# urw7rs/diffusion-models-made-easy

Hardware: AMD Instinct MI355X
Metric: denoising steps/sec + training images/sec, DDPM UNet CIFAR10 32×32 @1/2/4/8 GPU (higher is better)
Workload: dtype bf16; 1 GPU; DDPM T=1000 sampling, CIFAR10 32x32, default UNet (32,416,643 params, random init), batch 128 per GPU, t.shape=(1,); global_batch=128, parallelism=dp1 (independent chains per GPU, no data-path collective)

## Files before the change

diffusion-models-made-easy_amd/_lib.py:

```python

from __future__ import annotations

import ctypes as C
import os
import subprocess
import threading

_HERE = os.path.dirname(os.path.abspath(__file__))
LIB_PATH = os.environ.get("DMME_LIB_PATH") or os.path.join(_HERE, "libdmme_hip.so")
CSRC = os.path.join(_HERE, "csrc")

F16R32 = 4
F32, BF16, BF16X3, F16 = 0, 1, 2, 3
CHAIN_DDPM, CHAIN_DDIM, CHAIN_IDDPM, CHAIN_DDPM_GUIDED, CHAIN_DDIM_GUIDED, CHAIN_GDDIM = 0, 1, 2, 3, 4, 5
CHAIN_DDPM_CFG, CHAIN_GDDIM_CFG = 6, 7
CHAIN_DPMPP, CHAIN_DPMPP_CFG = 8, 9
CHAIN_REPAINT = 10
CHAIN_ILVR = 11
PRED_EPS, PRED_X0, PRED_V = 0, 1, 2
PREDICTIONS = {"eps": PRED_EPS, "x0": PRED_X0, "v": PRED_V}
THRESHOLD_NONE, THRESHOLD_STATIC, THRESHOLD_DYNAMIC = 0, 1, 2
THRESHOLDS = {"none": THRESHOLD_NONE, "static": THRESHOLD_STATIC, "dynamic": THRESHOLD_DYNAMIC}
ARCH_DDPM, ARCH_IDDPM, ARCH_CLASSIFIER, ARCH_DDPM_COND = 0, 1, 2, 3
DTYPES = {"fp32": F32, "float32": F32, "32": F32, "bf16": BF16, "bfloat16": BF16, "16": BF16, "bf16-mixed": BF16, "16-mixed": BF16,
# ... 93 lines not shown
    "dmme_unet_plan_check": (_i, [_vp]),
    "dmme_debug_level_stamps": (_i, [_vp, _i, _i]),
    "dmme_unet_plan_op_info": (_i, [_vp, _i, C.c_char_p, _i, C.POINTER(C.c_double), C.POINTER(C.c_double)]),
    "dmme_unet_forward_profiled": (_i, [_vp, _vp, _vp, _vp, _i, _vp, _vp, _vp, _vp, _vp]),
    "dmme_unet_plan_packed_bwd_bytes": (_i64, [_vp]),
    "dmme_unet_plan_bwd_workspace_bytes": (_i64, [_vp]),
    "dmme_unet_pack_params_bwd": (_i, [_vp, _vp, _vp, _vp]),
    "dmme_unet_backward": (_i, [_vp, _vp, _vp, _vp, _vp, _i, _vp, _vp, _vp, _vp, _vp, _vp, _vp]),
    "dmme_unet_backward_buckets": (_i, [_vp, _vp, _vp, _vp, _vp, _i, _vp, _vp, _vp, _vp, _vp, _vp, _vp, BUCKET_FN, _vp]),
    "dmme_unet_backward_input": (_i, [_vp, _vp, _vp, _vp, _vp, _i, _vp, _vp, _vp, _vp, _vp, _vp]),
    "dmme_unet_plan_grad_buckets": (_i, [_vp, C.POINTER(_i64), C.POINTER(_i64), C.POINTER(_i), _i]),
    "dmme_unet_plan_bwd_summary": (_i, [_vp, C.c_char_p, _i]),
    "dmme_grad_norm": (_i, [_vp, _i64, _vp, _vp, _vp]),
    "dmme_adam_step": (_i, [_vp, _vp, _vp, _vp, _vp, _i64, _f, _f, _f, _f, _i, _vp, _f, _f, _f, _vp]),
    "dmme_amp_init": (_i, [_vp, _f, _vp]),
    "dmme_amp_scale": (_i, [_vp, _i64, _vp, _vp]),
    "dmme_adam_step_amp": (_i, [_vp, _vp, _vp, _vp, _vp, _i64, _f, _f, _f, _f, _vp, _f, _f, _f, _vp, _f, _f, _i, _vp]),
    "dmme_grad_pack_bf16": (_i, [_vp, _i64, _vp, _i64, _vp]),
    "dmme_shard_reduce_bf16": (_i, [_vp, _i, _i64, _f, _vp, _vp]),
    "dmme_grad_unpack_bf16": (_i, [_vp, _i64, _vp, _vp]),
    "dmme_unet_debug_read": (_i, [_vp, _vp, C.c_char_p, _vp, _i64, C.POINTER(_i64), _vp]),
    "dmme_unet_debug_read_grad": (_i, [_vp, _vp, C.c_char_p, _vp, _i64, C.POINTER(_i64), _vp]),
    "dmme_unet_debug_read_norm_stats": (_i, [_vp, _vp, C.c_char_p, _vp, _i64, C.POINTER(_i64), _vp]),
    "dmme_dropout_masks": (_i, [_vp, _u64, _u64, _vp, _vp]),
    "dmme_randn": (_i, [_vp, _i64, _u64, _u64, _vp]),
    "dmme_q_sample": (_i, [_vp, _vp, _vp, _vp, _vp, _i, _i64, _vp, _vp, _vp]),
    "dmme_ddpm_step": (_i, [_vp, _vp, _vp, _f, _f, _f, _i, _i64, _vp]),
    "dmme_ddim_step": (_i, [_vp, _vp, _f, _f, _i64, _vp]),
    "dmme_gddim_step": (_i, [_vp, _vp, _vp, _f, _f, _f, _i64, _vp]),
    "dmme_slerp": (_i, [_vp, _vp, _vp, _i, _i, _i64, _vp, _vp]),
    "dmme_chain_set": (_i, [_vp, _i64, _vp, _u64, _u64, _vp]),
    "dmme_chain_update": (_i, [_i, _vp, _vp, _vp, _vp, _vp, _i, _i64, _vp]),
    "dmme_chain_step": (_i, [_vp, _vp, _vp, _vp, _vp, _i, _vp, _vp, _vp, _vp]),
    "dmme_chain_update_gddim": (_i, [_vp, _vp, _vp, _vp, _vp, _vp, _i, _i64, _vp]),
    "dmme_log_softmax_grad": (_i, [_vp, _vp, _i, _i, _i, _f, _vp, _vp, _vp, _vp]),
    "dmme_chain_update_guided": (_i, [_i, _vp, _vp, _vp, _vp, _vp, _vp, _vp, _i, _i64, _vp]),
    "dmme_guided_chain_step": (_i, [_vp, _vp, _vp, _vp, _vp, _vp, _vp, _vp, _vp, _vp, _vp, _vp, _vp, _vp, _vp, _i, _vp, _vp, _vp, _vp]),
    "dmme_mse_loss": (_i, [_vp, _vp, _i64, _vp, _vp, _f, _vp, _vp]),
    "dmme_pred_to_eps": (_i, [_i, _vp, _vp, _vp, _i, _vp, _i, _i, _i64, _vp]),
    "dmme_unet_plan_set_prediction": (_i, [_vp, _i, _vp, _i]),
    "dmme_x0_threshold": (_i, [_i, _vp, _vp, _vp, _i, _vp, _i, _i, _i64, _i, _i, _f, _i, _f, _vp, _vp]),
    "dmme_x0_threshold_scratch_bytes": (_i64, [_i, _i64]),
    "dmme_x0_threshold_lds_capacity": (_i, []),
    "dmme_unet_plan_set_threshold": (_i, [_vp, _i, _vp, _i, _i, _f, _vp]),
    "dmme_q_sample_pred": (_i, [_i, _vp, _vp, _vp, _vp, _vp, _i, _i64, _vp, _vp, _vp]),
    "dmme_mse_loss_rows": (_i, [_vp, _vp, _vp, _vp, _i, _i64, _vp, _vp, _f, _vp, _vp]),
# ... 96 lines not shown
```

diffusion-models-made-easy_amd/csrc/common.h:

```cpp
#pragma once

#include <hip/hip_runtime.h>
#include <stdint.h>

#include "dmme_hip.h"

namespace dmme {

void set_error(const char* fmt, ...) __attribute__((format(printf, 1, 2)));

int debug_route(const char* key, int dflt = 0);

#define DMME_CHECK_HIP(expr)                                                                          \
    do {                                                                                              \
        hipError_t e_ = (expr);                                                                       \
        if (e_ != hipSuccess) {                                                                       \
            ::dmme::set_error("%s failed: %s (%s:%d)", #expr, hipGetErrorString(e_), __FILE__, __LINE__); \
            return DMME_ERR_HIP;                                                                      \
        }                                                                                             \
    } while (0)

#define DMME_REQUIRE(cond, code, ...)        \
    do {                                     \
        if (!(cond)) {                       \
// ... 148 lines not shown
    const void* res1;
    const void* res2;
    void* dst;
    int N, Hin, Win, C1, C2;
    int up, stride, taps;
    int Hout, Wout, Cout;
    int pro_silu, out_silu;
    int nt, tproj_ld, R1;
    int in_nchw, out_nchw;
    float* gn_part;
    int gn_cg, gn_tiles;
    int gn_raw_moments;
    long long* stamps;
    float* splitk;
    int64_t splitk_cap;
    int x3;
    int mix;
    int mix2;
    int f16;
    int dma_b;
    GnOut gno[2];
    int n_gno;
    float gn_eps;
    void* act;
    int act_k, act_silu;
    const float* act_dmask;
    GnIn gni;
    int has_gni;
    const void* r_src1;
    const void* r_src2;
    const void* r_w;
    const float* r_bias;
    int r_C1, r_C2;
};

int launch_mfma_valu(int mode, int iters, int blocks, float* sink, hipStream_t s);
int launch_issue_probe(int kind, int n_inner, int iters, int flags, int blocks, long long* sink, const void* src, hipStream_t s);
int launch_l2_stream(const void* buf, int64_t bytes, int iters, int mode, int depth, int blocks, unsigned* sink, hipStream_t s);

struct ConvTile {
    int TW, TH, TN;
    int HH, HWd;
    int tiles_x, tiles_y;
    int tiles_m, tiles_n;
    int a_rows;
    unsigned magic_px, magic_w;
};
enum ConvFamily {
    CONV_GENERIC = 0,
// ... 325 lines not shown
```

diffusion-models-made-easy_amd/csrc/conv_common.h:

```cpp
#pragma once
#include <stdlib.h>

#include "common.h"

namespace dmme {

typedef float f32x16 __attribute__((ext_vector_type(16)));
typedef float f32x4 __attribute__((ext_vector_type(4)));
typedef __bf16 bf16x8 __attribute__((ext_vector_type(8)));
typedef f16 f16x8 __attribute__((ext_vector_type(8)));
template <typename T>
struct Vec8 {
    typedef T type __attribute__((ext_vector_type(8)));
};
template <typename T>
__device__ __forceinline__ void unpack8(const uint4& raw, float (&v)[8]) {
    const typename Vec8<T>::type x = __builtin_bit_cast(typename Vec8<T>::type, raw);
#pragma unroll
    for (int e = 0; e < 8; ++e) v[e] = (float)x[e];
}
template <typename T>
__device__ __forceinline__ uint4 pack8(const float (&v)[8]) {
    typename Vec8<T>::type x;
#pragma unroll
// ... 779 lines not shown
            float na = 0.f, mean = 0.f, m2 = 0.f;
            for (int j = 0; j < f; ++j) {
                const float* q = img + (tn * VPR + gi * f + j) * 2;
                const float delta = q[0] - mean, tot = na + cv;
                const float rt = __builtin_amdgcn_rcpf(tot);
                mean += delta * (cv * rt);
                m2 += q[1] + delta * delta * (na * cv * rt);
                na = tot;
            }
            const float rstd = 1.0f / sqrtf(m2 / na + a.gn_eps);
            for (int j = 0; j < f; ++j) {
                float* o = mr + (k * 256 + tn * VPR + gi * f + j) * 2;
                o[0] = mean;
                o[1] = rstd;
            }
            if (n0 + tn < a.N && G.mean_rstd) {
                float* o = G.mean_rstd + ((int64_t)(n0 + tn) * (G.C / G.cg) + (G.c_off + co0) / G.cg + gi) * 2;
                o[0] = mean;
                o[1] = rstd;
            }
        }
    }
    __syncthreads();
    for (int idx = tid; idx < TN * BN; idx += NT) {
        const int tn = idx / BN, c = idx % BN;
#pragma unroll
        for (int k = 0; k < 2; ++k) {
            if (k >= a.n_gno) break;
            const GnOut& G = a.gno[k];
            const float* q = mr + (k * 256 + tn * VPR + c / VEC) * 2;
            const int cc = G.c_off + co0 + c;
            const float gm = idx == tid ? gm0[k] : G.gamma[cc], bt = idx == tid ? bt0[k] : G.beta[cc];
            const float sc = q[1] * gm, sh = bt - q[0] * sc;
            if (n0 + tn < a.N) {
                G.scale[(int64_t)(n0 + tn) * G.C + cc] = sc;
                G.shift[(int64_t)(n0 + tn) * G.C + cc] = sh;
            }
            if (a.act && k == a.act_k) {
                ssc[idx] = sc;
                ssh[idx] = sh;
            }
        }
    }
    if (!a.act) return;
    __syncthreads();
    const GnOut& GA = a.gno[a.act_k];
    T* __restrict__ act = (T*)a.act;
#pragma unroll
    for (int q = 0; q < ITEMS; ++q) {
        const int it = tid + q * NT, m = it / VPR;
        const int opix = pix_of(m);
        if (opix < 0) continue;
        const int tn = m >> sh_hw;
        const float* dm = a.act_dmask ? a.act_dmask + (int64_t)(n0 + tn) * GA.C + GA.c_off + co0 + vec * VEC : nullptr;
        const uint4 o = prologue_vec<T>(kept[q], ssc + tn * BN + vec * VEC, ssh + tn * BN + vec * VEC, dm, a.act_silu);
        *reinterpret_cast<uint4*>(act + (int64_t)opix * GA.C + GA.c_off + co0 + vec * VEC) = o;
    }
}

template <typename T, int BM, int BN, int MI, int NI, int NT = 256, typename PixFn>
__device__ __forceinline__ void conv_epilogue(const ConvArgs& a, f32x16 (&acc)[MI][NI], int co0, int wn0, int r, int h,
                                              int wm0, int n0, int TN, PixFn pix_of, float* stage, int tile_s) {
    if (conv_epilogue_is_staged<T>(a, TN)) {
        conv_epilogue_stage<T, BN, MI, NI>(a, acc, co0, wn0, r, h, wm0, n0, stage);
        __syncthreads();
        conv_epilogue_store<T, BM, BN, NT>(a, co0, n0, pix_of, stage, tile_s);
        return;
    }
#pragma unroll
    for (int ni = 0; ni < NI; ++ni) {
        const int co = co0 + wn0 + ni * 32 + r;
        if (co >= a.Cout) continue;
        const float bias = a.bias ? a.bias[co] : 0.f;
#pragma unroll
        for (int mi = 0; mi < MI; ++mi) {
#pragma unroll
            for (int j = 0; j < 16; ++j) {
                const int m = wm0 + mi * 32 + (j & 3) + 8 * (j >> 2) + 4 * h;
                const int opix = pix_of(m);
// ... 62 lines not shown
```

diffusion-models-made-easy_amd/csrc/plan.h:

```cpp
#pragma once
#include <stdarg.h>
#include <stdlib.h>
#include <stdio.h>
#include <string.h>

#include <algorithm>
#include <memory>
#include <string>
#include <unordered_map>
#include <vector>

#include "common.h"
#include "lvl.h"

namespace dmme {

static inline int64_t align_up(int64_t v, int64_t a) { return (v + a - 1) / a * a; }

template <typename T>
class DevTable {
    T* p_ = nullptr;

public:
    DevTable() = default;
// ... 65 lines not shown
    int64_t lin_pre = -1;
    int gn_src1 = -1, gn_src2 = -1, gn_gamma = -1, gn_beta = -1;
    int64_t b_rowsum = 0, b_ab = 0;
    int64_t b_gnrows = -1;
    int gn_rows_deferred = 0;
    int64_t gn_scale = 0, gn_shift = 0, gn_mr = 0;
    int gn_mod_col = -1, gn_mod_C = 0;
    int64_t gn_act = -1;
    int gn_force_small = 0;
    int gn_consumer = -1;
    int gn_direct = 0;
    int gn_in_consumer = 0;
    int src1 = -1, src2 = -1;
    int w = -1, b = -1;
    int gn = -1;
    int pro_silu = 0, out_silu = 0;
    int64_t dmask_off = -1;
    int tproj_col = -1;
    int res1 = -1, res2 = -1;
    int dst = -1;
    int up = 0, stride = 1, taps = 9;
    int use_act = 0;
    int gd_n = 0, gd_gn[2] = {-1, -1}, gd_coff[2] = {0, 0};
    int gd_act = -1;
    int res_alias = 0;
    int rseg = -1, fused_away = 0;
    int wg_layer = -1;
    int64_t wg_act = -1;
    int bias_deferred = 0;
    int at_qkv = -1, at_out = -1, at_heads = 1;
    int64_t at_lse = 0;
    int at_proj = -1;
    int at_fold_qkv = -1;
    int folded_into = -1;
    int64_t fold_M = -1, fold_c = -1, fold_wpv = -1, fold_b2 = -1;
    int mix = 0, route_f32 = 0;
    int mix2 = 0;
    int cast_src = -1, cast_dst = -1;
    int lvl = -1, lvl_first = 0;
};

struct LvlRun {
    int op_first = 0, op_last = 0;
    int sh = 0, NG = 0, NGS = 0, GB = 1, NJ = 1;
    std::vector<LvlOp> ops;
    std::vector<std::pair<int, int>> made;
    DevTable<LvlOp> ops_dev;
// ... 108 lines not shown
```

diffusion-models-made-easy_amd/csrc/plan.hip:

```cpp
#include "plan.h"

#include <functional>
#include <map>
#include <mutex>

namespace dmme {

static thread_local char g_err[512] = "";
void set_error(const char* fmt, ...) {
    va_list ap;
    va_start(ap, fmt);
    vsnprintf(g_err, sizeof(g_err), fmt, ap);
    va_end(ap);
}

int debug_route(const char* key, int dflt) {
    const char* e = getenv("DMME_DEBUG_ROUTE");
    if (!e || !*e) return dflt;
    const size_t kl = strlen(key);
    for (const char* p = e; *p;) {
        const char* end = strchr(p, ',');
        const size_t len = end ? (size_t)(end - p) : strlen(p);
        if (len >= kl && !strncmp(p, key, kl) && (len == kl || p[kl] == '=')) return len == kl ? 1 : atoi(p + kl + 1);
        if (!end) break;
// ... 645 lines not shown
        a.res1 = ws + P->tensors[o.res1].off;
        a.R1 = P->tensors[o.res1].C;
        if (o.res2 >= 0) a.res2 = ws + P->tensors[o.res2].off;
    }
    if (P->splitk_floats > 0 && ws) {
        a.splitk = (float*)(ws + P->ws_splitk);
        a.splitk_cap = P->splitk_floats;
    }
    if (fwd && o.gd_n > 0) {
        a.n_gno = o.gd_n;
        a.gn_eps = 1e-5f;
        a.gn_cg = P->tensors[o.dst].C / P->cfg.num_groups;
        for (int k = 0; k < o.gd_n; ++k) {
            const Op& g = P->ops[o.gd_gn[k]];
            GnOut& G = a.gno[k];
            G.gamma = (const float*)(packed + P->params[g.gn_gamma].packed_off);
            G.beta = (const float*)(packed + P->params[g.gn_beta].packed_off);
            G.scale = (float*)(ws + g.gn_scale);
            G.shift = (float*)(ws + g.gn_shift);
            G.mean_rstd = (float*)(ws + g.gn_mr);
            G.C = P->tensors[g.gn_src1].C + (g.gn_src2 >= 0 ? P->tensors[g.gn_src2].C : 0);
            G.cg = G.C / P->cfg.num_groups;
            G.c_off = o.gd_coff[k];
            if (k == o.gd_act) {
                const Op& cv = P->ops[g.gn_consumer];
                a.act = ws + g.gn_act;
                a.act_k = k;
                a.act_silu = cv.pro_silu;
                a.act_dmask = (cv.dmask_off >= 0 && drop_masks) ? drop_masks + cv.dmask_off : nullptr;
            }
        }
    }
    a.gn_raw_moments = P->mix ? 1 : 0;
    if (o.dst == -2) {
        a.dst = y;
        a.out_nchw = 1;
    } else {
        const Tensor& td = P->tensors[o.dst];
        a.dst = ws + td.off;
        if (td.stats_off >= 0) {
            a.gn_part = (float*)(ws + td.stats_off);
            a.gn_cg = td.C / P->cfg.num_groups;
            a.gn_tiles = td.stats_tiles;
        }
    }
}

bool gn_from_parts(const dmme_plan* P, const Op& o) {
    if (o.gn_force_small) return false;
    const Tensor& t1 = P->tensors[o.gn_src1];
    if (t1.stats_off < 0) return false;
    const int G = P->cfg.num_groups;
// ... 83 lines not shown
            }
        }
    }
    int64_t ws = P->ws_bytes;
    const int64_t es = (int64_t)dtype_size(P->dtype);
    for (int t = 0; t < nT; ++t) {
        if (!elig[t]) continue;
        Op& o = P->ops[producer[t]];
        P->tensors[t].stats_off = -1;
        o.gd_n = (int)uses[t].size();
        for (int k = 0; k < o.gd_n; ++k) {
            o.gd_gn[k] = uses[t][k].gn;
            o.gd_coff[k] = uses[t][k].coff;
            P->ops[uses[t][k].gn].gn_direct = 1;
        }
    }
    if (getenv("DMME_NO_PREACT")) return;
    for (int ci = 0; ci < nO; ++ci) {
        Op& cv = P->ops[ci];
        if (cv.kind != OP_CONV || cv.gn < 0 || cv.src1 < 0 || cv.up || cv.stride != 1 || cv.lvl >= 0) continue;
        Op& g = P->ops[cv.gn];
        if (!g.gn_direct || g.gn_src2 >= 0 || g.gn_act >= 0 || g.gn_src1 != cv.src1 || cv.src2 >= 0) continue;
        Op& pr = P->ops[producer[g.gn_src1]];
        if (pr.gd_act >= 0 || elig[g.gn_src1] != 1) continue;
        for (int k = 0; k < pr.gd_n; ++k)
            if (pr.gd_gn[k] == cv.gn) pr.gd_act = k;
        if (pr.gd_act < 0) continue;
        const Tensor& t1 = P->tensors[g.gn_src1];
        g.gn_act = ws;
        g.gn_consumer = ci;
        cv.use_act = 1;
        ws = align_up(ws + (int64_t)P->B * t1.H * t1.W * t1.C * es, 256);
    }
    P->ws_bytes = ws;
}

void assign_preact(dmme_plan* P) {
    int64_t ws = P->ws_bytes;
    const int64_t es = (int64_t)dtype_size(P->dtype);
    for (int ci = 0; ci < (int)P->ops.size(); ++ci) {
        Op& cv = P->ops[ci];
        if (cv.kind != OP_CONV || cv.gn < 0 || cv.src1 < 0 || cv.up || cv.stride != 1 || cv.lvl >= 0) continue;
        Op& g = P->ops[cv.gn];
        constexpr bool over_parts = false;
        if (g.gn_mod_col >= 0 || g.gn_act >= 0 || g.gn_direct) continue;
        const Tensor& t1 = P->tensors[g.gn_src1];
        const int C2 = g.gn_src2 >= 0 ? P->tensors[g.gn_src2].C : 0;
        if (g.gn_src1 != cv.src1 || g.gn_src2 != cv.src2) continue;
        if (!gn_small_act_supported(P->dtype, t1.H * t1.W, t1.C, C2, P->cfg.num_groups)) continue;
        if (gn_from_parts(P, g)) {
// ... 423 lines not shown
    if (!P->fold_jobs.empty()) DMME_TRY(P->fold_jobs_dev.upload(P->fold_jobs));
    std::vector<dmme_plan::WgGroup*> all_groups{&P->wg[0], &P->wg[1], &P->wg[2]};
    for (auto& B_ : P->gb)
        for (int k = 0; k < 3; ++k) all_groups.push_back(&B_.wg[k]);
    for (dmme_plan::WgGroup* G : all_groups) {
        if (G->jobs.empty()) continue;
        DMME_TRY(G->layers_dev.upload(G->layers));
        DMME_TRY(G->jobs_dev.upload(G->jobs));
    }
    DMME_TRY(P->err_host.alloc());
    for (LvlRun& R : P->lvl_runs) {
        DMME_TRY(R.ops_dev.upload(R.ops));
        if (R.raw_skipped > 0) DMME_TRY(R.ops_nograd_dev.upload(R.ops_nograd));
        DMME_TRY(R.sync_dev.zeroed(16 + R.ops.size() * 2 * (size_t)R.NG * LVL_NS));
    }
    return DMME_OK;
}

}

extern "C" {

DMME_API const char* dmme_last_error(void) { return g_err; }
DMME_API int dmme_version(void) { return 116; }
DMME_API int dmme_device_count(void) {
    int n = 0;
    if (hipGetDeviceCount(&n) != hipSuccess) return 0;
    return n;
}

DMME_API int dmme_unet_plan_create(const dmme_unet_cfg* cfg, int B, int H, int W, int dtype, int device, dmme_plan** out) {
    DMME_REQUIRE(cfg && out, DMME_ERR_INVALID, "plan_create: null argument");
    DMME_TRY(check_cfg(cfg, B, H, W, dtype));
    std::unique_ptr<dmme_plan> owned(new dmme_plan());
    dmme_plan* P = owned.get();
    P->cfg = *cfg;
    if (cfg->arch == DMME_ARCH_DDPM_COND) {
        P->cond = 1;
        P->cfg.arch = DMME_ARCH_DDPM;
    }
    P->B = B;
    P->H = H;
    P->W = W;
    P->x3 = dtype == DMME_BF16X3;
    P->mix = dtype == DMME_F16R32;
    P->dtype = P->x3 ? DMME_F32 : P->mix ? DMME_F16 : dtype;
    P->device = device;
// ... 224 lines not shown
    const Tensor& t = plan->tensors[it->second];
    const int64_t n = (int64_t)plan->B * t.C * t.H * t.W;
    DMME_REQUIRE(n <= numel_cap, DMME_ERR_INVALID, "debug_read_grad: destination too small (%lld > %lld)", (long long)n,
                 (long long)numel_cap);
    if (numel_out) *numel_out = n;
    return launch_nhwc_to_nchw(plan->dtype, (const char*)bwd_workspace + plan->gt_off[it->second], plan->B, t.C, t.H * t.W, dst,
                               (hipStream_t)stream);
}

DMME_API int dmme_unet_debug_read_norm_stats(const dmme_plan* plan, const void* workspace, const char* name, float* dst,
                                             int64_t numel_cap, int64_t* numel_out, void* stream) {
    DMME_REQUIRE(plan && workspace && name && dst, DMME_ERR_INVALID, "debug_read_norm_stats: null argument");
    const std::string key = std::string(name) + ".weight";
    for (const Op& o : plan->ops) {
        if (o.kind != OP_GN || o.gn_gamma < 0 || plan->params[o.gn_gamma].name != key) continue;
        const int64_t n = (int64_t)plan->B * plan->cfg.num_groups * 2;
        DMME_REQUIRE(n <= numel_cap, DMME_ERR_INVALID, "debug_read_norm_stats: destination too small (%lld > %lld)", (long long)n,
                     (long long)numel_cap);
        DMME_CHECK_HIP(hipMemcpyAsync(dst, (const char*)workspace + o.gn_mr, (size_t)n * 4, hipMemcpyDeviceToDevice, (hipStream_t)stream));
        if (numel_out) *numel_out = n;
        return DMME_OK;
    }
    set_error("debug_read_norm_stats: no GroupNorm named '%s'", name);
    return DMME_ERR_INVALID;
}

DMME_API int dmme_dropout_masks(const dmme_plan* plan, uint64_t seed, uint64_t offset, float* masks, void* stream) {
    DMME_REQUIRE(plan && masks, DMME_ERR_INVALID, "dropout_masks: null argument");
    return launch_dropmask(masks, plan->dropmask_numel, plan->cfg.dropout, seed, offset, (hipStream_t)stream);
}

DMME_API int dmme_randn(float* out, int64_t numel, uint64_t seed, uint64_t offset, void* stream) {
    DMME_REQUIRE(out && numel >= 0, DMME_ERR_INVALID, "randn: bad argument");
    return launch_randn(out, numel, seed, offset, (hipStream_t)stream);
}

DMME_API int dmme_q_sample(const float* x0, const float* z, const float* sqrt_abar, const float* sqrt_1m_abar,
                           const int64_t* t, int B, int64_t chw, float* x_t, float* target, void* stream) {
    DMME_REQUIRE(x0 && z && sqrt_abar && sqrt_1m_abar && t && x_t && B > 0 && chw > 0, DMME_ERR_INVALID, "q_sample: bad argument");
    return launch_q_sample(x0, z, sqrt_abar, sqrt_1m_abar, t, B, chw, x_t, target, (hipStream_t)stream);
}

static SamplerOperands sampler_operands(float* x, const float* out, const float* zin, int64_t B, int64_t chw, const float* grad = nullptr,
                                        float* hist = nullptr, int planes = 1, const float* known = nullptr, const float* mask = nullptr) {
    return SamplerOperands{x, out, grad, zin, hist, known, mask, chw, B * chw, (B * chw + 3) / 4, planes};
}
// ... 484 lines not shown
```

diffusion-models-made-easy_amd/csrc/plan_lvl.hip:

```cpp
#include "plan.h"

using namespace dmme;

namespace dmme {

static int op_level(const dmme_plan* P, const Op& o) {
    auto hw = [&](int id, int& H, int& W) {
        if (id < 0) return true;
        const Tensor& t = P->tensors[id];
        if (H == 0) {
            H = t.H;
            W = t.W;
            return true;
        }
        return t.H == H && t.W == W;
    };
    int H = 0, W = 0;
    bool ok = true;
    if (o.kind == OP_CONV) {
        if (o.src1 < 0 || o.dst < 0 || o.stride != 1 || o.up || (o.taps != 1 && o.taps != 9)) return 0;
        for (int id : {o.src1, o.src2, o.dst, o.res1, o.res2}) ok = ok && hw(id, H, W);
    } else if (o.kind == OP_GN) {
        ok = hw(o.gn_src1, H, W) && hw(o.gn_src2, H, W);
    } else if (o.kind == OP_ATTN) {
        ok = hw(o.at_qkv, H, W) && hw(o.at_out, H, W);
    } else {
        return 0;
    }
    if (!ok || H != W || (H != 4 && H != 8)) return 0;
    return H;
}

struct LvlXAttach {
    int run, op;
    LvlNorm norm;
};
static bool build_lvl_run(dmme_plan* P, int i0, int i1, int lvl_w, int64_t& ws, LvlRun& R, std::vector<std::pair<int, int64_t>>& gn_acts,
                          const std::unordered_map<int, std::pair<int, int>>& made, std::vector<LvlXAttach>& xattach) {
    const int B = P->B, G = P->cfg.num_groups, HW = lvl_w * lvl_w;
    const int64_t es = (int64_t)dtype_size(P->dtype);
    std::vector<LvlOp> pre, body;
    std::unordered_map<int, int> prod;
    std::unordered_map<int, int> pre_of;
    std::vector<int> xsrc;
    const bool merge_res_off = (debug_route("lvl_no_res_merge") != 0);
    auto is_x = [&](int t) { return std::find(xsrc.begin(), xsrc.end(), t) != xsrc.end(); };
    auto row_of = [&](int tensor) -> int {
        auto it = prod.find(tensor);
        if (it != prod.end()) return 1000000 + it->second * 2;
        auto jt = pre_of.find(tensor);
        if (jt != pre_of.end()) return jt->second * 2;
        return -1;
    };
    auto blank = [&]() {
        LvlOp o{};
        o.kind = LVL_CONV;
        o.taps = 1;
        o.wait0 = o.wait1 = o.wait2 = o.wait3 = -1;
        o.a1_off = o.a2_off = o.a3_off = o.a4_off = o.dst_off = o.res_off = o.sc_off = -1;
        o.w2_off = o.b2_off = -1;
        o.tproj_col = -1;
// ... 23 lines not shown
            const int64_t act = ws;
            ws = align_up(ws + (int64_t)B * HW * Cn * es, 256);
            gn_acts.push_back({oi, act});
            int coff = 0;
            for (int src : {o.gn_src1, o.gn_src2}) {
                if (src < 0) continue;
                LvlNorm n{};
                n.gamma_off = P->params[o.gn_gamma].packed_off;
                n.beta_off = P->params[o.gn_beta].packed_off;
                n.scale_off = o.gn_scale;
                n.shift_off = o.gn_shift;
                n.mr_off = o.gn_mr;
                n.act_off = act;
                n.dmask_off = cv.dmask_off;
                n.Cn = Cn;
                n.cg = cg;
                n.c_off = coff;
                n.act_silu = cv.pro_silu;
                LvlOp* host = nullptr;
                auto it = prod.find(src);
                auto mt = made.find(src);
                if (it != prod.end()) {
                    host = &body[it->second];
                } else if (mt != made.end() && pre_of.find(src) == pre_of.end()) {
                    int used = P->lvl_runs[mt->second.first].ops[mt->second.second].n_norm;
                    for (const LvlXAttach& xa : xattach) used += xa.run == mt->second.first && xa.op == mt->second.second;
                    if (used >= 2) return false;
                    xattach.push_back({mt->second.first, mt->second.second, n});
                    xsrc.push_back(src);
                    coff += P->tensors[src].C;
                    continue;
                } else {
                    auto jt = pre_of.find(src);
                    if (jt == pre_of.end()) {
                        LvlOp q = blank();
                        q.kind = LVL_NORM;
                        q.dst_off = P->tensors[src].off;
                        q.dst_C = P->tensors[src].C;
                        q.dst_c0 = 0;
                        pre_of[src] = (int)pre.size();
                        pre.push_back(q);
                        jt = pre_of.find(src);
                    }
                    host = &pre[jt->second];
                }
                if (host->n_norm >= 2) return false;
// ... 92 lines not shown
                q.reuse_a = j > 0;
                if (j > 0) q.wait0 = q.wait1 = -1;
                body.push_back(q);
            }
            prod[o.dst] = (int)body.size() - 1;
        } else {
            prod[o.dst] = (int)body.size();
            body.push_back(c);
        }
    }
    const int shift = (int)pre.size();
    R.ops = pre;
    for (LvlOp c : body) {
        for (int* wr : {&c.wait0, &c.wait1, &c.wait2, &c.wait3})
            if (*wr >= 1000000) *wr = (*wr - 1000000) + shift * 2;
        R.ops.push_back(c);
    }
    R.made.clear();
    for (auto& kv : pre_of) R.made.push_back({kv.first, kv.second});
    for (auto& kv : prod) R.made.push_back({kv.first, kv.second + shift});
    return !body.empty();
}

void assign_levels(dmme_plan* P) {
    if (getenv("DMME_NO_LVL") || P->cfg.arch != DMME_ARCH_DDPM || P->x3 || (P->dtype != DMME_BF16 && P->dtype != DMME_F16)) return;
    const int mask = debug_route("lvl_mask", 12);
    if (P->device >= 0) {
        const int n = lvl_engine_max_resident(P->dtype, P->device);
        if (n < LVL_NS) return;
        P->lvl_max_wg = n;
    }
    if (debug_route("lvl_max_wg", 0) > 0) P->lvl_max_wg = std::min(P->lvl_max_wg, debug_route("lvl_max_wg", 0));
    if (P->lvl_max_wg < LVL_NS) return;
    const int nO = (int)P->ops.size();
    std::unordered_map<int, std::pair<int, int>> made;
    int i = 0;
    while (i < nO) {
        const int L = op_level(P, P->ops[i]);
        if (!L) {
            ++i;
            continue;
        }
        int j = i;
        while (j < nO && op_level(P, P->ops[j]) == L) ++j;
        if (mask & L) {
            LvlRun R;
            R.op_first = i;
            R.op_last = j - 1;
            R.sh = L == 4 ? 2 : 3;
            R.NG = (P->B * L * L + LVL_BM - 1) / LVL_BM;
            int64_t ws = P->ws_bytes;
            std::vector<std::pair<int, int64_t>> gn_acts;
            std::vector<LvlXAttach> xattach;
            if (build_lvl_run(P, i, j, L, ws, R, gn_acts, debug_route("lvl_no_xrun") ? std::unordered_map<int, std::pair<int, int>>() : made, xattach)) {
                bool has_attn = false;
                for (const LvlOp& lo : R.ops) has_attn = has_attn || lo.kind == LVL_ATTN;
                int slots = P->lvl_max_wg / LVL_NS;
                R.GB = (R.NG > slots && !has_attn && !debug_route("lvl_gb1")) ? 2 : 1;
                const int nb = (R.NG + R.GB - 1) / R.GB;
                R.NJ = (R.GB == 2 && nb > slots && !debug_route("lvl_nj1")) ? 2 : 1;
                slots *= R.NJ;
                R.NGS = nb < slots ? nb : slots;
                const int max_iter = debug_route("lvl_max_iter", 2);
                if ((nb + slots - 1) / slots > max_iter) {
                    i = j;
                    continue;
                }
                P->ws_bytes = ws;
                for (const LvlXAttach& xa : xattach) {
                    LvlOp& host = P->lvl_runs[xa.run].ops[xa.op];
                    host.norm[host.n_norm++] = xa.norm;
                }
                for (auto& mk : R.made) made[mk.first] = {(int)P->lvl_runs.size(), mk.second};
                const int ri = (int)P->lvl_runs.size();
                for (int oi = i; oi < j; ++oi) {
                    Op& o = P->ops[oi];
                    o.lvl = ri;
                    o.lvl_first = oi == i;
                    if (o.kind == OP_GN) o.gn_direct = 1;
                }
                for (auto& ga : gn_acts) {
                    Op& g = P->ops[ga.first];
                    g.gn_act = ga.second;
                    for (int ci = ga.first + 1; ci < j; ++ci)
                        if (P->ops[ci].kind == OP_CONV && P->ops[ci].gn == ga.first) {
                            g.gn_consumer = ci;
                            P->ops[ci].use_act = 1;
                        }
                }
                P->lvl_runs.push_back(std::move(R));
            }
        }
        i = j;
    }
}

void assign_lvl_nograd(dmme_plan* P) {
    if (P->lvl_runs.empty()) return;
    std::vector<char> need(P->tensors.size(), 0);
    auto mark = [&](int id) { if (id >= 0) need[id] = 1; };
    for (const Op& q : P->ops) {
        if (q.kind == OP_CONV) {
            if (!(q.gn >= 0 && q.use_act)) { mark(q.src1); mark(q.src2); }
            mark(q.res1);
            mark(q.res2);
        } else if (q.kind == OP_GN) {
            for (int id : {q.gn_src1, q.gn_src2}) {
                if (id < 0) continue;
                if (q.lvl < 0) { need[id] = 1; continue; }
                for (const LvlOp& lo : P->lvl_runs[q.lvl].ops)
                    if (lo.kind == LVL_NORM && lo.dst_off == P->tensors[id].off) need[id] = 1;
            }
        } else if (q.kind == OP_ATTN) {
            if (q.lvl < 0) mark(q.at_qkv);
        } else if (q.kind == OP_CAST) {
            mark(q.cast_src);
// ... 125 lines not shown
```

diffusion-models-made-easy_amd/models/ddpm.py:

```python

from __future__ import annotations

import ctypes as C
import weakref
from typing import Dict, Optional, Sequence, Tuple

import torch
from torch import Tensor, nn

from .. import _lib


class _Scope(nn.Module):
    """Parameter container used to reproduce the reference's dotted state_dict keys."""


def _cfg_struct(in_channels, pos_dim, emb_dim, num_groups, dropout, channels_per_depth, num_blocks, attention_depths, arch=0, num_heads=1,
                num_classes=0):
    cfg = _lib.UNetCfg()
    cfg.arch, cfg.num_heads, cfg.num_classes = int(arch), int(num_heads), int(num_classes)
    cfg.in_channels, cfg.pos_dim, cfg.emb_dim, cfg.num_groups = in_channels, pos_dim, emb_dim, num_groups
    cfg.dropout = float(dropout)
    if not 1 <= len(channels_per_depth) <= 8 or len(attention_depths) > 8:
        raise ValueError("channels_per_depth must have 1..8 entries and attention_depths at most 8")
# ... 471 lines not shown

    def check_engine(self):
        torch.cuda.synchronize()
        for plan in self._plans.values():
            plan.check()

    def debug_activation(self, name: str) -> Tensor:
        plan = self._last_plan
        cap = plan.B * 4096 * max(plan.H * plan.W, 1)
        buf = torch.empty(cap, dtype=torch.float32, device=plan.workspace.device)
        n = C.c_int64()
        _lib.check(plan.lib.dmme_unet_debug_read(plan.h, _lib.ptr(plan.workspace), name.encode(), _lib.ptr(buf), cap, C.byref(n), _lib.stream_ptr()), "dmme_unet_debug_read")
        return buf[: n.value].clone()

    def debug_norm_stats(self, name: str) -> Tensor:
        plan = self._last_plan
        G = int(self._cfg.num_groups)
        buf = torch.empty(plan.B * G * 2, dtype=torch.float32, device=plan.workspace.device)
        n = C.c_int64()
        _lib.check(plan.lib.dmme_unet_debug_read_norm_stats(plan.h, _lib.ptr(plan.workspace), name.encode(), _lib.ptr(buf), buf.numel(), C.byref(n),
                                                            _lib.stream_ptr()), "dmme_unet_debug_read_norm_stats")
        return buf[: n.value].view(plan.B, G, 2).clone()

    def debug_gradient(self, name: str) -> Tensor:
        plan = self._last_plan
        if getattr(plan, "bws", None) is None:
            raise RuntimeError("debug_gradient: no backward pass has run on this plan")
        cap = plan.B * 4096 * max(plan.H * plan.W, 1)
        buf = torch.empty(cap, dtype=torch.float32, device=plan.bws.device)
        n = C.c_int64()
        _lib.check(plan.lib.dmme_unet_debug_read_grad(plan.h, _lib.ptr(plan.bws), name.encode(), _lib.ptr(buf), cap, C.byref(n), _lib.stream_ptr()),
                   "dmme_unet_debug_read_grad")
        return buf[: n.value].clone()
```

include/dmme_hip.h:

```cpp
#ifndef DMME_HIP_H
#define DMME_HIP_H

#include <stddef.h>
#include <stdint.h>

#if defined(DMME_BUILD)
#define DMME_API __attribute__((visibility("default")))
#else
#define DMME_API
#endif

#ifdef __cplusplus
extern "C" {
#endif

typedef enum {
    DMME_OK = 0,
    DMME_ERR_INVALID = -1,
    DMME_ERR_UNSUPPORTED = -2,
    DMME_ERR_HIP = -3,
    DMME_ERR_NOMEM = -4
} dmme_status;

typedef enum { DMME_F32 = 0, DMME_BF16 = 1, DMME_BF16X3 = 2, DMME_F16 = 3, DMME_F16R32 = 4 } dmme_dtype;
// ... 86 lines not shown
DMME_API int dmme_debug_level_stamps(void* buf, int run, int workgroup);
DMME_API int dmme_debug_mfma_valu(int mode, int iters, int blocks, void* sink, void* stream);
DMME_API int dmme_debug_issue_probe(int kind, int n_inner, int iters, int flags, int blocks, void* sink, const void* src, void* stream);
DMME_API int dmme_debug_l2_stream(const void* buf, int64_t bytes, int iters, int mode, int depth, int blocks, void* sink, void* stream);
DMME_API int dmme_grad_norm(const float* grad, int64_t numel, float* norm_out, float* scratch, void* stream);
DMME_API int dmme_adam_step(float* param, const float* grad, float* exp_avg, float* exp_avg_sq, float* ema, int64_t numel,
                            float lr, float beta1, float beta2, float eps, int step, const float* grad_norm, float max_norm,
                            float ema_decay, float grad_scale, void* stream);
DMME_API int dmme_amp_init(float* amp_state, float init_scale, void* stream);
DMME_API int dmme_amp_scale(float* grad, int64_t numel, const float* amp_state, void* stream);
DMME_API int dmme_adam_step_amp(float* param, const float* grad, float* exp_avg, float* exp_avg_sq, float* ema, int64_t numel, float lr, float beta1,
                                float beta2, float eps, const float* grad_norm, float max_grad_norm, float ema_decay, float grad_scale,
                                float* amp_state, float growth_factor, float backoff_factor, int growth_interval, void* stream);
DMME_API int dmme_grad_pack_bf16(const float* grad, int64_t numel, void* dst_bf16, int64_t numel_padded, void* stream);
DMME_API int dmme_shard_reduce_bf16(const void* recv_bf16, int world, int64_t per_rank, float scale, void* out_bf16, void* stream);
DMME_API int dmme_grad_unpack_bf16(const void* src_bf16, int64_t numel, float* grad, void* stream);

DMME_API int dmme_unet_debug_read(const dmme_plan* plan, const void* workspace, const char* name, float* dst,
                         int64_t numel_cap, int64_t* numel_out, void* stream);
DMME_API int dmme_unet_debug_read_grad(const dmme_plan* plan, const void* bwd_workspace, const char* name, float* dst,
                         int64_t numel_cap, int64_t* numel_out, void* stream);
DMME_API int dmme_unet_debug_read_norm_stats(const dmme_plan* plan, const void* workspace, const char* name, float* dst,
                         int64_t numel_cap, int64_t* numel_out, void* stream);


DMME_API int dmme_dropout_masks(const dmme_plan* plan, uint64_t seed, uint64_t offset, float* masks, void* stream);


DMME_API int dmme_randn(float* out, int64_t numel, uint64_t seed, uint64_t offset, void* stream);

DMME_API int dmme_q_sample(const float* x0, const float* z, const float* sqrt_abar, const float* sqrt_1m_abar,
                  const int64_t* t, int B, int64_t chw, float* x_t, float* target, void* stream);

DMME_API int dmme_ddpm_step(float* x, const float* eps, const float* z, float inv_sqrt_alpha, float eps_coef,
                   float sigma, int add_noise, int64_t numel, void* stream);

DMME_API int dmme_ddim_step(float* x, const float* eps, float sqrt_one_minus_abar, float sqrt_abar_prev, int64_t numel,
                   void* stream);

DMME_API int dmme_gddim_step(float* x, const float* eps, const float* z, float k0, float k1, float k2, int64_t numel, void* stream);

DMME_API int dmme_slerp(const float* xa, const float* xb, const float* w, int n, int B, int64_t chw, float* out, void* stream);

DMME_API int dmme_mse_loss(const float* eps, const float* target, int64_t numel, float* loss, float* d_eps,
                  float grad_scale, float* scratch, void* stream);

// ... 165 lines not shown
```

Before: 480.1 denoising steps/s (one step = UNet forward + DDPM update on a batch of 128), summed over GPUs.

## Fuse GroupNorm stats and activation writes into border convs feeding level runs

Convolutions outside level runs whose outputs feed GroupNorms inside level runs now compute the GroupNorm statistics directly in their epilogue and write normalized activations for up to two consumers (act arrays, gd_act bitmask). Level-run building treats these border tensors as external inputs, and the plan rebuilds without the change if any consumer fails to pick up the fused activation. Attention level runs whose block count exceeds the available slots are also skipped. The intent is to remove separate GroupNorm passes and extra activation reads at level boundaries, at the cost of a more complex epilogue with extra syncs and a second plan build.

```diff
diff --git a/diffusion-models-made-easy_amd/_lib.py b/diffusion-models-made-easy_amd/_lib.py
--- a/diffusion-models-made-easy_amd/_lib.py
+++ b/diffusion-models-made-easy_amd/_lib.py
@@ -139,6 +139,7 @@
     "dmme_unet_debug_read": (_i, [_vp, _vp, C.c_char_p, _vp, _i64, C.POINTER(_i64), _vp]),
     "dmme_unet_debug_read_grad": (_i, [_vp, _vp, C.c_char_p, _vp, _i64, C.POINTER(_i64), _vp]),
     "dmme_unet_debug_read_norm_stats": (_i, [_vp, _vp, C.c_char_p, _vp, _i64, C.POINTER(_i64), _vp]),
+    "dmme_unet_debug_read_norm_rows": (_i, [_vp, _vp, C.c_char_p, _vp, _i64, C.POINTER(_i64), _vp]),
     "dmme_dropout_masks": (_i, [_vp, _u64, _u64, _vp, _vp]),
     "dmme_randn": (_i, [_vp, _i64, _u64, _u64, _vp]),
     "dmme_q_sample": (_i, [_vp, _vp, _vp, _vp, _vp, _i, _i64, _vp, _vp, _vp]),
diff --git a/diffusion-models-made-easy_amd/csrc/common.h b/diffusion-models-made-easy_amd/csrc/common.h
--- a/diffusion-models-made-easy_amd/csrc/common.h
+++ b/diffusion-models-made-easy_amd/csrc/common.h
@@ -194,9 +194,9 @@
     GnOut gno[2];
     int n_gno;
     float gn_eps;
-    void* act;
-    int act_k, act_silu;
-    const float* act_dmask;
+    void* act[2];
+    int act_silu[2];
+    const float* act_dmask[2];
     GnIn gni;
     int has_gni;
     const void* r_src1;
diff --git a/diffusion-models-made-easy_amd/csrc/conv_common.h b/diffusion-models-made-easy_amd/csrc/conv_common.h
--- a/diffusion-models-made-easy_amd/csrc/conv_common.h
+++ b/diffusion-models-made-easy_amd/csrc/conv_common.h
@@ -825,12 +825,13 @@
         }
     }
     __syncthreads();
-    for (int idx = tid; idx < TN * BN; idx += NT) {
-        const int tn = idx / BN, c = idx % BN;
-#pragma unroll
-        for (int k = 0; k < 2; ++k) {
-            if (k >= a.n_gno) break;
-            const GnOut& G = a.gno[k];
+#pragma unroll
+    for (int k = 0; k < 2; ++k) {
+        if (k >= a.n_gno) break;
+        const GnOut& G = a.gno[k];
+        T* __restrict__ act = (T*)a.act[k];
+        for (int idx = tid; idx < TN * BN; idx += NT) {
+            const int tn = idx / BN, c = idx % BN;
             const float* q = mr + (k * 256 + tn * VPR + c / VEC) * 2;
             const int cc = G.c_off + co0 + c;
             const float gm = idx == tid ? gm0[k] : G.gamma[cc], bt = idx == tid ? bt0[k] : G.beta[cc];
@@ -839,25 +840,24 @@
                 G.scale[(int64_t)(n0 + tn) * G.C + cc] = sc;
                 G.shift[(int64_t)(n0 + tn) * G.C + cc] = sh;
             }
-            if (a.act && k == a.act_k) {
+            if (act) {
                 ssc[idx] = sc;
                 ssh[idx] = sh;
             }
         }
-    }
-    if (!a.act) return;
-    __syncthreads();
-    const GnOut& GA = a.gno[a.act_k];
-    T* __restrict__ act = (T*)a.act;
-#pragma unroll
-    for (int q = 0; q < ITEMS; ++q) {
-        const int it = tid + q * NT, m = it / VPR;
-        const int opix = pix_of(m);
-        if (opix < 0) continue;
-        const int tn = m >> sh_hw;
-        const float* dm = a.act_dmask ? a.act_dmask + (int64_t)(n0 + tn) * GA.C + GA.c_off + co0 + vec * VEC : nullptr;
-        const uint4 o = prologue_vec<T>(kept[q], ssc + tn * BN + vec * VEC, ssh + tn * BN + vec * VEC, dm, a.act_silu);
-        *reinterpret_cast<uint4*>(act + (int64_t)opix * GA.C + GA.c_off + co0 + vec * VEC) = o;
+        if (!act) continue;
+        __syncthreads();
+#pragma unroll
+        for (int q = 0; q < ITEMS; ++q) {
+            const int it = tid + q * NT, m = it / VPR;
+            const int opix = pix_of(m);
+            if (opix < 0) continue;
+            const int tn = m >> sh_hw;
+            const float* dm = a.act_dmask[k] ? a.act_dmask[k] + (int64_t)(n0 + tn) * G.C + G.c_off + co0 + vec * VEC : nullptr;
+            const uint4 o = prologue_vec<T>(kept[q], ssc + tn * BN + vec * VEC, ssh + tn * BN + vec * VEC, dm, a.act_silu[k]);
+            *reinterpret_cast<uint4*>(act + (int64_t)opix * G.C + G.c_off + co0 + vec * VEC) = o;
+        }
+        if (k == 0 && a.n_gno > 1 && a.act[1]) __syncthreads();
     }
 }
 
diff --git a/diffusion-models-made-easy_amd/csrc/plan.h b/diffusion-models-made-easy_amd/csrc/plan.h
--- a/diffusion-models-made-easy_amd/csrc/plan.h
+++ b/diffusion-models-made-easy_amd/csrc/plan.h
@@ -111,7 +111,7 @@
     int up = 0, stride = 1, taps = 9;
     int use_act = 0;
     int gd_n = 0, gd_gn[2] = {-1, -1}, gd_coff[2] = {0, 0};
-    int gd_act = -1;
+    int gd_act = 0;
     int res_alias = 0;
     int rseg = -1, fused_away = 0;
     int wg_layer = -1;
diff --git a/diffusion-models-made-easy_amd/csrc/plan.hip b/diffusion-models-made-easy_amd/csrc/plan.hip
--- a/diffusion-models-made-easy_amd/csrc/plan.hip
+++ b/diffusion-models-made-easy_amd/csrc/plan.hip
@@ -691,12 +691,11 @@
             G.C = P->tensors[g.gn_src1].C + (g.gn_src2 >= 0 ? P->tensors[g.gn_src2].C : 0);
             G.cg = G.C / P->cfg.num_groups;
             G.c_off = o.gd_coff[k];
-            if (k == o.gd_act) {
+            if (o.gd_act >> k & 1) {
                 const Op& cv = P->ops[g.gn_consumer];
-                a.act = ws + g.gn_act;
-                a.act_k = k;
-                a.act_silu = cv.pro_silu;
-                a.act_dmask = (cv.dmask_off >= 0 && drop_masks) ? drop_masks + cv.dmask_off : nullptr;
+                a.act[k] = ws + g.gn_act;
+                a.act_silu[k] = cv.pro_silu;
+                a.act_dmask[k] = (cv.dmask_off >= 0 && drop_masks) ? drop_masks + cv.dmask_off : nullptr;
             }
         }
     }
@@ -826,10 +825,10 @@
         Op& g = P->ops[cv.gn];
         if (!g.gn_direct || g.gn_src2 >= 0 || g.gn_act >= 0 || g.gn_src1 != cv.src1 || cv.src2 >= 0) continue;
         Op& pr = P->ops[producer[g.gn_src1]];
-        if (pr.gd_act >= 0 || elig[g.gn_src1] != 1) continue;
+        if (pr.gd_act || elig[g.gn_src1] != 1) continue;
         for (int k = 0; k < pr.gd_n; ++k)
-            if (pr.gd_gn[k] == cv.gn) pr.gd_act = k;
-        if (pr.gd_act < 0) continue;
+            if (pr.gd_gn[k] == cv.gn) pr.gd_act = 1 << k;
+        if (!pr.gd_act) continue;
         const Tensor& t1 = P->tensors[g.gn_src1];
         g.gn_act = ws;
         g.gn_consumer = ci;
@@ -1299,7 +1298,7 @@
 extern "C" {
 
 DMME_API const char* dmme_last_error(void) { return g_err; }
-DMME_API int dmme_version(void) { return 116; }
+DMME_API int dmme_version(void) { return 117; }
 DMME_API int dmme_device_count(void) {
     int n = 0;
     if (hipGetDeviceCount(&n) != hipSuccess) return 0;
@@ -1570,6 +1569,24 @@
         return DMME_OK;
     }
     set_error("debug_read_norm_stats: no GroupNorm named '%s'", name);
+    return DMME_ERR_INVALID;
+}
+
+DMME_API int dmme_unet_debug_read_norm_rows(const dmme_plan* plan, const void* workspace, const char* name, float* dst,
+                                            int64_t numel_cap, int64_t* numel_out, void* stream) {
+    DMME_REQUIRE(plan && workspace && name && dst, DMME_ERR_INVALID, "debug_read_norm_rows: null argument");
+    const std::string key = std::string(name) + ".weight";
+    for (const Op& o : plan->ops) {
+        if (o.kind != OP_GN || o.gn_gamma < 0 || plan->params[o.gn_gamma].name != key) continue;
+        const int64_t C = plan->tensors[o.gn_src1].C + (o.gn_src2 >= 0 ? plan->tensors[o.gn_src2].C : 0), n = (int64_t)plan->B * C;
+        DMME_REQUIRE(2 * n <= numel_cap, DMME_ERR_INVALID, "debug_read_norm_rows: destination too small (%lld > %lld)", (long long)(2 * n),
+                     (long long)numel_cap);
+        DMME_CHECK_HIP(hipMemcpyAsync(dst, (const char*)workspace + o.gn_scale, (size_t)n * 4, hipMemcpyDeviceToDevice, (hipStream_t)stream));
+        DMME_CHECK_HIP(hipMemcpyAsync(dst + n, (const char*)workspace + o.gn_shift, (size_t)n * 4, hipMemcpyDeviceToDevice, (hipStream_t)stream));
+        if (numel_out) *numel_out = 2 * n;
+        return DMME_OK;
+    }
+    set_error("debug_read_norm_rows: no GroupNorm named '%s'", name);
     return DMME_ERR_INVALID;
 }
 
diff --git a/diffusion-models-made-easy_amd/csrc/plan_lvl.hip b/diffusion-models-made-easy_amd/csrc/plan_lvl.hip
--- a/diffusion-models-made-easy_amd/csrc/plan_lvl.hip
+++ b/diffusion-models-made-easy_amd/csrc/plan_lvl.hip
@@ -36,7 +36,7 @@
     LvlNorm norm;
 };
 static bool build_lvl_run(dmme_plan* P, int i0, int i1, int lvl_w, int64_t& ws, LvlRun& R, std::vector<std::pair<int, int64_t>>& gn_acts,
-                          const std::unordered_map<int, std::pair<int, int>>& made, std::vector<LvlXAttach>& xattach) {
+                          const std::unordered_map<int, std::pair<int, int>>& made, std::vector<LvlXAttach>& xattach, const std::vector<char>* border) {
     const int B = P->B, G = P->cfg.num_groups, HW = lvl_w * lvl_w;
     const int64_t es = (int64_t)dtype_size(P->dtype);
     std::vector<LvlOp> pre, body;
@@ -106,6 +106,10 @@
                 auto mt = made.find(src);
                 if (it != prod.end()) {
                     host = &body[it->second];
+                } else if (border && (*border)[src]) {
+                    xsrc.push_back(src);
+                    coff += P->tensors[src].C;
+                    continue;
                 } else if (mt != made.end() && pre_of.find(src) == pre_of.end()) {
                     int used = P->lvl_runs[mt->second.first].ops[mt->second.second].n_norm;
                     for (const LvlXAttach& xa : xattach) used += xa.run == mt->second.first && xa.op == mt->second.second;
@@ -244,7 +248,7 @@
     return !body.empty();
 }
 
-void assign_levels(dmme_plan* P) {
+static void build_levels(dmme_plan* P, const std::vector<char>* border) {
     if (getenv("DMME_NO_LVL") || P->cfg.arch != DMME_ARCH_DDPM || P->x3 || (P->dtype != DMME_BF16 && P->dtype != DMME_F16)) return;
     const int mask = debug_route("lvl_mask", 12);
     if (P->device >= 0) {
@@ -274,12 +278,16 @@
             int64_t ws = P->ws_bytes;
             std::vector<std::pair<int, int64_t>> gn_acts;
             std::vector<LvlXAttach> xattach;
-            if (build_lvl_run(P, i, j, L, ws, R, gn_acts, debug_route("lvl_no_xrun") ? std::unordered_map<int, std::pair<int, int>>() : made, xattach)) {
+            if (build_lvl_run(P, i, j, L, ws, R, gn_acts, debug_route("lvl_no_xrun") ? std::unordered_map<int, std::pair<int, int>>() : made, xattach, border)) {
                 bool has_attn = false;
                 for (const LvlOp& lo : R.ops) has_attn = has_attn || lo.kind == LVL_ATTN;
                 int slots = P->lvl_max_wg / LVL_NS;
                 R.GB = (R.NG > slots && !has_attn && !debug_route("lvl_gb1")) ? 2 : 1;
                 const int nb = (R.NG + R.GB - 1) / R.GB;
+                if (has_attn && nb > slots) {
+                    i = j;
+                    continue;
+                }
                 R.NJ = (R.GB == 2 && nb > slots && !debug_route("lvl_nj1")) ? 2 : 1;
                 slots *= R.NJ;
                 R.NGS = nb < slots ? nb : slots;
@@ -314,6 +322,82 @@
             }
         }
         i = j;
+    }
+}
+
+constexpr int kLvlNormOpsDefault = 0;
+void assign_levels(dmme_plan* P) {
+    const std::vector<Op> ops0 = P->ops;
+    const int64_t ws0 = P->ws_bytes;
+    build_levels(P, nullptr);
+    const int keep_ops = debug_route("lvl_norm_ops", kLvlNormOpsDefault);
+    if (P->lvl_runs.empty() || (keep_ops & 1)) return;
+    const int nT = (int)P->tensors.size(), nO = (int)P->ops.size(), G = P->cfg.num_groups;
+    struct Use { int gn, coff; };
+    std::vector<std::vector<Use>> uses(nT);
+    std::vector<char> outside(nT, 0);
+    for (int oi = 0; oi < nO; ++oi) {
+        const Op& g = P->ops[oi];
+        if (g.kind != OP_GN) continue;
+        int coff = 0;
+        for (int src : {g.gn_src1, g.gn_src2}) {
+            if (src < 0) continue;
+            if (g.lvl >= 0) uses[src].push_back({oi, coff});
+            else outside[src] = 1;
+            coff += P->tensors[src].C;
+        }
+    }
+    std::vector<int> producer(nT, -1);
+    std::vector<char> border(nT, 0);
+    bool any = false;
+    for (int oi = 0; oi < nO; ++oi) {
+        const Op& o = P->ops[oi];
+        if (o.kind != OP_CONV || o.dst < 0 || o.lvl >= 0) continue;
+        const int t = o.dst;
+        if (uses[t].empty() || uses[t].size() > 2 || outside[t] || P->tensors[t].C % G || (keep_ops & P->tensors[t].H)) continue;
+        ConvArgs a{};
+        fill_conv(P, o, (const char*)4096, (const float*)4096, (float*)4096, (char*)4096, nullptr, 1, a);
+        a.nt = o.tproj_col >= 0 ? P->B : 0;
+        a.gn_part = nullptr;
+        a.n_gno = (int)uses[t].size();
+        a.gn_cg = P->tensors[t].C / G;
+        bool ok = true;
+        int cgs[2] = {0, 0};
+        for (size_t k = 0; k < uses[t].size(); ++k) {
+            const Op& g = P->ops[uses[t][k].gn];
+            const int C = P->tensors[g.gn_src1].C + (g.gn_src2 >= 0 ? P->tensors[g.gn_src2].C : 0);
+            if (g.gn_mod_col >= 0 || C % G || uses[t][k].coff % (C / G)) ok = false;
+            cgs[k] = C / G;
+        }
+        if (!ok || conv_gn_direct_query(conv_dt(P, o), a, cgs, a.n_gno) != 1) continue;
+        producer[t] = oi;
+        border[t] = 1;
+        any = true;
+    }
+    if (!any) return;
+    auto rebuild = [&](const std::vector<char>* b) {
+        P->ops = ops0;
+        P->ws_bytes = ws0;
+        P->lvl_runs.clear();
+        build_levels(P, b);
+    };
+    rebuild(&border);
+    for (int t = 0; t < nT && any; ++t)
+        for (const Use& u : uses[t])
+            if (border[t] && (P->ops[u.gn].lvl < 0 || P->ops[u.gn].gn_act < 0)) any = false;
+    if (!any) {
+        rebuild(nullptr);
+        return;
+    }
+    for (int t = 0; t < nT; ++t) {
+        if (!border[t]) continue;
+        Op& o = P->ops[producer[t]];
+        o.gd_n = (int)uses[t].size();
+        for (int k = 0; k < o.gd_n; ++k) {
+            o.gd_gn[k] = uses[t][k].gn;
+            o.gd_coff[k] = uses[t][k].coff;
+            o.gd_act |= 1 << k;
+        }
     }
 }
 
diff --git a/diffusion-models-made-easy_amd/models/ddpm.py b/diffusion-models-made-easy_amd/models/ddpm.py
--- a/diffusion-models-made-easy_amd/models/ddpm.py
+++ b/diffusion-models-made-easy_amd/models/ddpm.py
@@ -517,6 +517,14 @@
                                                             _lib.stream_ptr()), "dmme_unet_debug_read_norm_stats")
         return buf[: n.value].view(plan.B, G, 2).clone()
 
+    def debug_norm_rows(self, name: str) -> Tensor:
+        plan = self._last_plan
+        buf = torch.empty(plan.B * 2 * 4096, dtype=torch.float32, device=plan.workspace.device)
+        n = C.c_int64()
+        _lib.check(plan.lib.dmme_unet_debug_read_norm_rows(plan.h, _lib.ptr(plan.workspace), name.encode(), _lib.ptr(buf), buf.numel(), C.byref(n),
+                                                           _lib.stream_ptr()), "dmme_unet_debug_read_norm_rows")
+        return buf[: n.value].view(2, plan.B, -1).clone()
+
     def debug_gradient(self, name: str) -> Tensor:
         plan = self._last_plan
         if getattr(plan, "bws", None) is None:
diff --git a/include/dmme_hip.h b/include/dmme_hip.h
--- a/include/dmme_hip.h
+++ b/include/dmme_hip.h
@@ -132,6 +132,8 @@
                          int64_t numel_cap, int64_t* numel_out, void* stream);
 DMME_API int dmme_unet_debug_read_norm_stats(const dmme_plan* plan, const void* workspace, const char* name, float* dst,
                          int64_t numel_cap, int64_t* numel_out, void* stream);
+DMME_API int dmme_unet_debug_read_norm_rows(const dmme_plan* plan, const void* workspace, const char* name, float* dst,
+                         int64_t numel_cap, int64_t* numel_out, void* stream);
 
 
 DMME_API int dmme_dropout_masks(const dmme_plan* plan, uint64_t seed, uint64_t offset, float* masks, void* stream);
```

New measurement: 482.4 denoising steps/s (one step = UNet forward + DDPM update on a batch of 128), summed over GPUs (median of 6 runs). No clear change (+0.5%).
